# cbiffle/rtiow-rust

Hardware: AMD Instinct MI355X
Metric: Msamples/s (pixels*spp/s), book-1 random-spheres 1200x800 (higher is better)
Workload: dtype f32

## Files before the change

rtiow-rust_amd/capi.py:

```python
import ctypes as C
import math
import os
import time

import numpy as np

from . import noise

c_f32p = C.POINTER(C.c_float)
c_u32p = C.POINTER(C.c_uint32)
c_u8p = C.POINTER(C.c_uint8)

INVALID_ID = 0xFFFFFFFF
FLAG_COUNTERS = 1
FLAG_TRACE_KERNEL = 2
FLAG_PARTIAL = 4
FLAG_RESUME = 8
FLAG_SUM_SQUARES = 16
FLAG_SAMPLE_COUNTS = 32
FLAG_RETIRE = 64
RETIRE_MAX_RADIUS = 8
FLAG_DENOISE = 128
DENOISE_MAX_RADIUS = 8
DENOISE_MAX_PATCH = 3
# ... 471 lines not shown
        f("object_translate", C.c_uint32, [C.c_void_p, c_f32p, C.c_uint32])
        f("object_scale", C.c_uint32, [C.c_void_p, c_f32p, C.c_uint32])
        f("object_rotate_y", C.c_uint32, [C.c_void_p, C.c_float, C.c_uint32])
        f("object_and", C.c_uint32, [C.c_void_p, C.c_uint32, C.c_uint32])
        f("object_rect_prism", C.c_uint32, [C.c_void_p, c_f32p, c_f32p, C.c_uint32])
        f("object_linear_move", C.c_uint32, [C.c_void_p, C.c_uint32, c_f32p])
        f("object_constant_medium", C.c_uint32, [C.c_void_p, C.c_uint32, C.c_float, C.c_uint32])
        f("object_bvh", C.c_uint32, [C.c_void_p, c_u32p, C.c_size_t, C.c_float, C.c_float])
        f("object_bvh_sah", C.c_uint32, [C.c_void_p, c_u32p, C.c_size_t, C.c_float, C.c_float])
        f("camera_look", C.c_int, [c_f32p, c_f32p, c_f32p] + [C.c_float] * 6 + [C.POINTER(Camera)])
        f("scene_create", C.c_int, [C.c_void_p, c_u32p, C.c_size_t, C.c_int, C.POINTER(C.c_void_p)])
        f("scene_destroy", None, [C.c_void_p])
        self._declare_render()
        f("debug_hit_top", C.c_int, [C.c_void_p, C.c_size_t, c_f32p, C.c_uint64, C.c_float, c_f32p, c_u32p])
        f("debug_samples", C.c_int, [C.c_void_p, C.POINTER(Camera), C.POINTER(Params), C.c_size_t,
                                     c_u32p, c_u32p, c_u32p, c_f32p, c_u32p])
        f("debug_math", C.c_int, [C.c_int, C.c_int, C.c_size_t, c_f32p, c_f32p, c_f32p])
        f("tonemap", C.c_int, [C.c_int, C.c_size_t, c_f32p, c_u8p])

    def _declare_render(self):
        f = self._fn
        f("device_count", C.c_int, [C.POINTER(C.c_int)])
        f("scene_set_option", C.c_int, [C.c_void_p, C.c_char_p, C.c_int])
        f("scene_info", C.c_int, [C.c_void_p, c_u32p, c_u32p, c_u32p, C.POINTER(C.c_uint64), c_u32p])
        f("par_cast", C.c_int, [C.c_void_p, C.POINTER(Camera), C.POINTER(Params), c_f32p, C.POINTER(Stats)])
        f("par_cast_device", C.c_int, [C.c_void_p, C.POINTER(Camera), C.POINTER(Params), C.c_void_p,
                                       C.c_void_p, C.POINTER(Stats)])
        f("par_cast_multi", C.c_int, [C.POINTER(C.c_void_p), C.c_int, C.POINTER(Camera), C.POINTER(Params), c_f32p,
                                      C.POINTER(Stats)])
        f("multi_reset", C.c_int, [C.c_char_p, C.POINTER(C.c_uint64)])
        f("debug_flatten", C.c_int, [C.c_void_p, c_u32p, C.c_size_t, c_u32p, c_u32p, c_u32p, C.c_size_t])
        f("debug_flatten_pool2", C.c_int, [C.c_void_p, c_u32p, C.c_size_t, c_u32p, c_u32p, c_u32p, C.c_size_t])
        f("tonemap_device", C.c_int, [C.c_int, C.c_size_t, C.c_void_p, C.c_void_p, C.c_void_p])

    def _fn(self, name, restype, argtypes):
        try:
            fn = getattr(self.lib, self.prefix + name)
        except AttributeError:
            def fn(*_a, _n=self.prefix + name):
                raise RtError(ERR_INVALID, "%s: symbol %s is not exported by this build" % (self.path, _n))
            setattr(self, "_" + name, fn)
            return fn
        fn.restype = restype
        fn.argtypes = argtypes
        setattr(self, "_" + name, fn)
        return fn

    def last_error(self):
        return (self._last_error() or b"").decode()

    def check(self, code):
        if code != 0:
            raise RtError(code, self.last_error())

    def check_id(self, i):
        if i == INVALID_ID:
            raise RtError(-1, self.last_error())
        return i

    def builder(self):
        return Builder(self)

    def device_count(self):
        n = C.c_int(0)
        self.check(self._device_count(C.byref(n)))
        return n.value
# ... 129 lines not shown
    def rect_prism(self, p0, p1, material):
        return self.be.check_id(self.be._object_rect_prism(self.h, _f3(p0), _f3(p1), material))

    def linear_move(self, obj, motion):
        return self.be.check_id(self.be._object_linear_move(self.h, obj, _f3(motion)))

    def constant_medium(self, boundary, density, material):
        return self.be.check_id(self.be._object_constant_medium(self.h, boundary, density, material))

    def bvh(self, objs, exposure=(0.0, 1.0)):
        arr = (C.c_uint32 * max(1, len(objs)))(*objs)
        return self.be.check_id(self.be._object_bvh(self.h, arr, len(objs), exposure[0], exposure[1]))

    def flatten(self, world):
        arr = (C.c_uint32 * max(1, len(world)))(*world)
        n, feat = C.c_uint32(), C.c_uint32()
        self.be.check(self.be._debug_flatten(self.h, arr, len(world), C.byref(n), C.byref(feat), None, 0))
        words = np.zeros((n.value, 8), dtype=np.uint32)
        self.be.check(self.be._debug_flatten(self.h, arr, len(world), C.byref(n), C.byref(feat),
                                             words.ctypes.data_as(c_u32p), n.value))
        return words, feat.value

    def flatten_pool2(self, world):
        arr = (C.c_uint32 * max(1, len(world)))(*world)
        n = C.c_uint32()
        table = np.zeros(24, dtype=np.uint32)
        self.be.check(self.be._debug_flatten_pool2(self.h, arr, len(world), C.byref(n), table.ctypes.data_as(c_u32p), None, 0))
        words = np.zeros((n.value, 8), dtype=np.uint32)
        self.be.check(self.be._debug_flatten_pool2(self.h, arr, len(world), C.byref(n), table.ctypes.data_as(c_u32p),
                                                   words.ctypes.data_as(c_u32p), n.value))
        items = [tuple(int(v) for v in table[4 * k:4 * k + 4]) for k in range(int(table[20]))]
        return words, items, int(table[21]), int(table[22])

    def bvh_sah(self, objs, exposure=(0.0, 1.0)):
        arr = (C.c_uint32 * max(1, len(objs)))(*objs)
        return self.be.check_id(self.be._object_bvh_sah(self.h, arr, len(objs), exposure[0], exposure[1]))

    def scene(self, world, device=0):
        arr = (C.c_uint32 * max(1, len(world)))(*world)
        h = C.c_void_p()
        self.be.check(self.be._scene_create(self.h, arr, len(world), device, C.byref(h)))
        sc = self.be.scene_class(self.be, h, self)
        sc.apply_env_options()
        return sc


class Scene:
    def __init__(self, backend, handle, builder):
        self.be = backend
        self.h = handle
        self._builder = builder

    def close(self):
        if self.h:
            self.be._scene_destroy(self.h)
            self.h = None

    def __del__(self):
        try:
            self.close()
        except Exception:
            pass

    ENV_OPTIONS = ("kernel", "chunks", "lpt", "lpt_phase1", "lpt_deep", "lpt_shift", "ray_lds", "sync", "block", "wg_per_cu", "window",
                   "box_leave", "refill_min", "gather_min", "run_ahead", "run_ahead_min", "sphere_min", "verbose", "bvh4", "box_chains", "force_rccl", "multi_gather", "multi_planes", "scratch_mb", "frames_in_flight", "small_frames", "drain_share", "hoist", "deep_sized", "mat_lds", "pool2", "p2_refill", "p2_box_leave", "p2_park", "p2_sphere", "p2_prism", "p2_list", "p2_push")

    def set_option(self, name, value):
        self.be.check(self.be._scene_set_option(self.h, name.encode(), int(value)))

    def apply_env_options(self):
        if not hasattr(self.be, "_scene_set_option"):
            return
        for name in self.ENV_OPTIONS:
            v = os.environ.get("RTG_" + name.upper())
            if v is not None:
                self.set_option(name, int(v))

    def info(self):
        a, b, c, d, e = C.c_uint32(), C.c_uint32(), C.c_uint32(), C.c_uint64(), C.c_uint32()
        self.be.check(self.be._scene_info(self.h, C.byref(a), C.byref(b), C.byref(c), C.byref(d), C.byref(e)))
        return {"instructions": a.value, "materials": b.value, "textures": c.value, "hbm_bytes": d.value, "box_followers": e.value}

    def _par_cast_args(self, args, threads):
        return args

    def par_cast(self, camera, nx, ny, ns, seed=0xDEADBEEF, stats=False, out=None, threads=0, counts=None, counters=None,
                 retire=None, denoise=None, features=None, **kw):
        def call(p, buf):
            st = Stats.new()
            self.be.check(self.be._par_cast(*self._par_cast_args(
                [self.h, C.byref(camera), C.byref(p), buf.ctypes.data_as(c_f32p), C.byref(st)], threads)))
            return st
        return _render(lambda part: _supported(self.be, part), call, nx, ny, ns, seed, stats, out,
                       stats if counters is None else counters, counts, retire, denoise, features, kw, exact=True)

    def par_cast_device(self, camera, params, d_out_ptr, stream=None, want_stats=False, sample_begin=None, partial=None,
                        resume=None, squares=None, counts=None, retire=None, denoise=None, features=None):
        over = {"squares": squares, "counts": counts, "retire": retire, "denoise": denoise, "features": features}
# ... 245 lines not shown
```

rtiow-rust_amd/csrc/rtg_api.hip:

```cpp
#include <hip/hip_runtime.h>

#include <dlfcn.h>
#include <rccl/rccl.h>

#include <cmath>
#include <cstdio>
#include <cstdlib>
#include <cstring>
#include <map>
#include <mutex>
#include <functional>
#include <string>
#include <tuple>
#include <vector>

#include "../../include/rtiow_gpu.h"
#include "rt_pool.h"
#include "rt_retire.h"
#include "rt_denoise.h"
#include "rt_features.h"
#include "rt_multi_planes.h"
#include "rt_pool_full.h"
#include "rt_sync_full.h"
#include "rt_pool2.h"
#include "rt_trace.h"
#include "scene_builder.h"

using namespace rtg;

#include "rtg_kernels.inc"

namespace {
thread_local std::string g_err;

int fail(int code, const std::string& msg) {
  g_err = msg;
  return code;
}
int hip_fail(hipError_t e, const char* what) {
  return fail(RTG_ERR_DEVICE, std::string(what) + ": " + hipGetErrorString(e));
}
#define HIP_TRY(expr)                                   \
  do {                                                  \
    hipError_t e_ = (expr);                             \
    if (e_ != hipSuccess) return hip_fail(e_, #expr);   \
  } while (0)
}

struct rtg_builder {
  SceneBuilder sb;
// ... 9 lines not shown
  size_t stack_bytes = 0;
  uint32_t* d_slots = nullptr;
  size_t slots_bytes = 0;
  float* d_scratch = nullptr;
  size_t scratch_bytes = 0;
  LaunchConsts* d_consts = nullptr;
  uint32_t* d_lpt = nullptr;
  size_t lpt_bytes = 0;
  LptQueue lpt_desc{};
  KernelKind last_kernel = KernelKind::baseline;
  uint32_t last_pix_work = 0;
  uint32_t* d_list = nullptr;
  size_t list_bytes = 0;
  uint32_t* d_compact = nullptr;
  size_t compact_bytes = 0;
  unsigned long long counts_samples = 0;
  void* d_retire = nullptr;
  size_t retire_bytes = 0;
  const char* refusal = nullptr;
  void* d_denoise = nullptr;
  size_t denoise_bytes = 0;
  rtg_denoise denoise_in{};
  uint32_t* d_features = nullptr;
  size_t features_bytes = 0;
  rtg_features features_in{};
};

struct rtg_scene {
  int device = 0;
  DevScene dev{};
  uint32_t features = 0;
  uint32_t n_prog = 0, n_mat = 0, n_tex = 0;
  uint64_t bytes = 0;
  void* buffers[13] = {nullptr, nullptr, nullptr, nullptr, nullptr, nullptr, nullptr, nullptr, nullptr, nullptr, nullptr, nullptr, nullptr};
  const uint32_t* d_parent = nullptr;
  hipStream_t own_stream = nullptr;
  int num_cus = 0;
  float* d_frame = nullptr;
  size_t frame_bytes = 0;
  int force_chunks = 0;
  uint64_t scratch_limit = 0;
  bool whole_scratch = false;
  int verbose = 0;
  int window = -1;
  int ray_lds = 1;
  int force_rccl = 0;
  int multi_gather = 0;
  float* d_pack = nullptr;
  size_t pack_bytes = 0;
  float* d_recv = nullptr;
  size_t recv_bytes = 0;
  int multi_planes = 0;
  hipEvent_t post0 = nullptr, post1 = nullptr;
  hipEvent_t pack0 = nullptr, pack1 = nullptr, unpack0 = nullptr;
  int bvh4 = 0;
  uint32_t wide_bytes = 0;
  int box_chains = 1;
  uint32_t n_followers = 0;
  const uint32_t* d_chain_off = nullptr;
  uint32_t chain_bytes = 0;
  int sync_full = -1;
  uint32_t n_box = 0;
  int lpt = 2;
  int lpt_deep = 4;
  int lpt_shift = 0;
  int lpt_phase1 = 0;
  int kernel_version = 3;
  PoolTuning pool_tune{40, 16, 24, 16, 16, 40};
  PoolTuning full_tune{20, 24, 32, 16, 24, 40};
  PoolTuning sync_tune{20, 16, 32, 16, 16, 40};
  int wg_per_cu = 0;
  int full_threads = 0;
  int pool_threads = 0;
  int mat_lds = 1;
  int deep_sized = 1;
  int hoist = 1;
  uint32_t seg_first = 0, seg_end = 0;
  int drain_share = 1;
  int pool2 = 1;
  uint32_t n_prog2 = 0, n_box2 = 0;
  DevScene dev2{};
  const P2Table* d_p2 = nullptr;
  Pool2Tuning pool2_tune{24, 48, 40, 4, 8, 24, 2};
  int guide_lds = 0;
  int small_frames = 1;
  LaunchCtx ctx[RTG_MAX_FRAMES];
  int n_ctx = 1, next_ctx = 0;
  LaunchCtx* cx = &ctx[0];
};

static void ctx_free_buffers(LaunchCtx* c) {
  if (c->busy) (void)hipEventSynchronize(c->done);
  c->busy = false;
// ... 311 lines not shown
  float theta = fov * 3.14159265358979323846f / 180.f;
  float half_height = tanf(theta / 2.f);
  float half_width = aspect * half_height;
  float w[3] = {from[0] - at[0], from[1] - at[1], from[2] - at[2]};
  unit(w);
  float u[3], v[3];
  cross3(up, w, u);
  unit(u);
  cross3(w, u, v);
  float hw_fd = half_width * focus_dist, hh_fd = half_height * focus_dist;
  float h2 = (2.f * half_width) * focus_dist, v2 = (2.f * half_height) * focus_dist;
  for (int i = 0; i < 3; i++) {
    out->origin[i] = from[i];
    out->lower_left_corner[i] = ((from[i] - hw_fd * u[i]) - hh_fd * v[i]) - focus_dist * w[i];
    out->horizontal[i] = h2 * u[i];
    out->vertical[i] = v2 * v[i];
    out->u[i] = u[i];
    out->v[i] = v[i];
  }
  out->lens_radius = lens_radius;
  out->exposure_start = e0;
  out->exposure_end = e1;
  return RTG_OK;
}

static int upload(void** dst, const void* src, size_t bytes, uint64_t* total) {
  size_t alloc = bytes ? bytes : 16;
  HIP_TRY(hipMalloc(dst, alloc));
  if (bytes) HIP_TRY(hipMemcpy(*dst, src, bytes, hipMemcpyHostToDevice));
  *total += alloc;
  return RTG_OK;
}

void rtg_scene_destroy(rtg_scene* s) {
  if (!s) return;
  (void)hipSetDevice(s->device);
  for (void* p : s->buffers)
    if (p) (void)hipFree(p);
  for (LaunchCtx& c : s->ctx) {
    ctx_free_buffers(&c);
    if (c.d_counters) (void)hipFree(c.d_counters);
    if (c.d_consts) (void)hipFree(c.d_consts);
    if (c.ev0) (void)hipEventDestroy(c.ev0);
    if (c.ev1) (void)hipEventDestroy(c.ev1);
    if (c.done) (void)hipEventDestroy(c.done);
  }
  if (s->d_frame) (void)hipFree(s->d_frame);
  if (s->d_pack) (void)hipFree(s->d_pack);
  if (s->d_recv) (void)hipFree(s->d_recv);
  if (s->post0) (void)hipEventDestroy(s->post0);
  if (s->post1) (void)hipEventDestroy(s->post1);
  for (hipEvent_t ev : {s->pack0, s->pack1, s->unpack0})
    if (ev) (void)hipEventDestroy(ev);
  if (s->own_stream) (void)hipStreamDestroy(s->own_stream);
  delete s;
}

int rtg_scene_create(rtg_builder* b, const rtg_id* world, size_t n, int device, rtg_scene** out) {
  if (!b || !out || (!world && n)) return fail(RTG_ERR_INVALID, "null argument");
  FlatScene fs;
  try {
    b->sb.flatten(world, n, &fs);
  } catch (const BuildError& e) {
    return fail(e.code, e.msg);
  }
  int ndev = 0;
// ... 45 lines not shown
  if (!fs.hi2.empty()) {
    if ((rc = upload(&s->buffers[9], fs.lo2.data(), fs.lo2.size() * 16, &s->bytes)) ||
        (rc = upload(&s->buffers[10], fs.hi2.data(), fs.hi2.size() * 16, &s->bytes)) ||
        (rc = upload(&s->buffers[11], &fs.p2, sizeof(P2Table), &s->bytes))) {
      rtg_scene_destroy(s);
      return rc;
    }
    s->dev2 = s->dev;
    s->dev2.lo = (const uint4*)s->buffers[9], s->dev2.hi = (const uint4*)s->buffers[10];
    s->dev2.n_prog = s->n_prog2 = (uint32_t)fs.hi2.size();
    s->dev2.lds_off = nullptr, s->dev2.lds_image_bytes = 0;
    s->d_p2 = (const P2Table*)s->buffers[11];
    for (const Packet& h : fs.hi2) s->n_box2 += (h.w[3] & 0xffu) == OP_BOX ? 1u : 0u;
  }
  if ((fs.features & (FEAT_ALL | FEAT_BOUNDARY)) == 0) {
    std::vector<uint32_t> ops(fs.hi.size()), off(fs.hi.size());
    for (size_t i = 0; i < fs.hi.size(); i++) ops[i] = fs.hi[i].w[3];
    s->dev.lds_image_bytes = lds_image_offsets(ops.data(), ops.size(), off.data());
    if ((rc = upload(&s->buffers[6], off.data(), off.size() * sizeof(uint32_t), &s->bytes))) {
      rtg_scene_destroy(s);
      return rc;
    }
    s->dev.lds_off = (const uint32_t*)s->buffers[6];
    std::vector<uint8_t> follower(fs.hi.size());
    s->n_followers = box_chain_followers(reinterpret_cast<const uint32_t (*)[4]>(fs.lo.data()), reinterpret_cast<const uint32_t (*)[4]>(fs.hi.data()), fs.hi.size(), follower.data());
    if (s->n_followers) {
      s->chain_bytes = lds_image_offsets(ops.data(), ops.size(), off.data(), follower.data());
      if ((rc = upload(&s->buffers[12], off.data(), off.size() * sizeof(uint32_t), &s->bytes))) {
        rtg_scene_destroy(s);
        return rc;
      }
      s->d_chain_off = (const uint32_t*)s->buffers[12];
    }
    std::vector<uint32_t> wide;
    if (build_wide_image(fs.lo.data(), fs.hi.data(), fs.hi.size(), wide)) {
      if ((rc = upload(&s->buffers[7], wide.data(), wide.size() * sizeof(uint32_t), &s->bytes))) {
        rtg_scene_destroy(s);
        return rc;
      }
      s->wide_bytes = (uint32_t)(wide.size() * sizeof(uint32_t));
    }
  }
  hipDeviceProp_t prop;
  if (hipGetDeviceProperties(&prop, device) == hipSuccess) s->num_cus = prop.multiProcessorCount;
  if (s->num_cus <= 0) s->num_cus = 256;
  if ((rc = ctx_acquire(s))) {
    rtg_scene_destroy(s);
    return rc;
  }
  s->next_ctx = 0;
  *out = s;
  return RTG_OK;
}


int rtg_scene_set_option(rtg_scene* s, const char* name, int value) {
  if (!s || !name) return fail(RTG_ERR_INVALID, "null argument");
  const std::string k(name);
  const uint32_t u = (uint32_t)value;
  if (k == "kernel") s->kernel_version = value;
  else if (k == "chunks") s->force_chunks = value;
  else if (k == "scratch_mb") s->scratch_limit = value > 0 ? (uint64_t)value << 20 : 0;
  else if (k == "lpt") s->lpt = value;
  else if (k == "lpt_phase1") s->lpt_phase1 = value;
  else if (k == "lpt_deep") s->lpt_deep = value;
  else if (k == "lpt_shift") s->lpt_shift = std::min(6, std::max(0, value));
  else if (k == "ray_lds") s->ray_lds = value;
  else if (k == "box_chains") s->box_chains = value;
  else if (k == "bvh4") {
    if (value && !s->wide_bytes) return fail(RTG_ERR_INVALID, "bvh4: the scene is not one Bvh of spheres (no 4-wide image)");
    if (value && pool_lds_bytes(s->wide_bytes, s->n_mat, (uint32_t)(s->pool_threads > 0 ? s->pool_threads : RT_POOL_MAX_THREADS) / 64u, true, false) > 160 * 1024)
      return fail(RTG_ERR_INVALID, "bvh4: the 4-wide image does not fit a CU's 160 KB of LDS (the 4-wide walk only exists LDS-staged)");
    s->bvh4 = value;
  }
  else if (k == "frames_in_flight") {
    if (value < 1 || value > RTG_MAX_FRAMES) return fail(RTG_ERR_INVALID, "frames_in_flight: 1 .. 4");
    HIP_TRY(hipSetDevice(s->device));
    for (int i = value; i < RTG_MAX_FRAMES; i++) ctx_free_buffers(&s->ctx[i]);
    s->n_ctx = value, s->next_ctx = 0;
  }
  else if (k == "force_rccl") s->force_rccl = value;
  else if (k == "multi_gather") s->multi_gather = value;
  else if (k == "multi_planes") s->multi_planes = value;
  else if (k == "sync") s->sync_full = value;
  else if (k == "block") {
    if (value < 64 || value > 1024 || value % 64) return fail(RTG_ERR_INVALID, "block: a multiple of 64 in [64, 1024]");
    s->pool_threads = s->full_threads = value;
  }
  else if (k == "wg_per_cu") s->wg_per_cu = value;
  else if (k == "drain_share") s->drain_share = value;
  else if (k == "hoist") s->hoist = value;
  else if (k == "pool2") s->pool2 = value;
  else if (k == "deep_sized") s->deep_sized = value;
  else if (k == "mat_lds") s->mat_lds = value;
  else if (k == "guide_lds") s->guide_lds = value;
  else if (k == "small_frames") s->small_frames = value;
  else if (k == "verbose") s->verbose = value;
  else if (k == "window") s->window = value;
  else if (k == "box_leave") s->pool_tune.box_leave = s->full_tune.box_leave = s->sync_tune.box_leave = u;
  else if (k == "refill_min") s->pool_tune.refill_min = s->full_tune.refill_min = s->sync_tune.refill_min = u;
  else if (k == "gather_min") s->pool_tune.gather_min = s->full_tune.gather_min = s->sync_tune.gather_min = u;
// ... 296 lines not shown
```

rtiow-rust_amd/csrc/rtg_launch.inc:

```
static uint64_t scratch_cap(int n_ctx) {
  size_t free_b = 0, total_b = 0;
  if (hipMemGetInfo(&free_b, &total_b) != hipSuccess) return (16ull << 30) / (uint64_t)std::max(1, n_ctx);
  return (uint64_t)free_b / 2 / (uint64_t)std::max(1, n_ctx);
}

static uint32_t samples_per_pass(const rtg_scene* s, uint64_t pix_work, uint32_t ns) {
  const uint64_t per_sample = pix_work * 3 * sizeof(float);
  uint64_t budget = s->scratch_limit ? s->scratch_limit : std::max<uint64_t>(scratch_cap(s->n_ctx), s->cx->scratch_bytes);
  if (s->whole_scratch) budget = ~0ull;
  uint64_t k = std::max<uint64_t>(1, budget / std::max<uint64_t>(per_sample, 1));
  k = std::min<uint64_t>(k, 0xfffffffeull / std::max<uint64_t>(pix_work, 1));
  k = std::max<uint64_t>(1, std::min<uint64_t>(k, ns));
  const uint64_t n_pass = (ns + k - 1) / k;
  return (uint32_t)((ns + n_pass - 1) / n_pass);
}

static uint64_t rank_pix_work(const DevParams& d) {
  const uint32_t tiles_x = (d.nx + d.tile_w - 1) / d.tile_w, tiles_y = (d.ny + d.tile_h - 1) / d.tile_h, tiles = tiles_x * tiles_y;
  const uint32_t owned = tiles > d.rank ? (tiles - d.rank + d.nranks - 1) / d.nranks : 0;
  return ((uint64_t)owned * d.tile_w * d.tile_h + 255u) & ~255ull;
}
static uint64_t owned_pixels(const DevParams& d) {
  uint64_t px = 0;
  uint32_t tiles_x = (d.nx + d.tile_w - 1) / d.tile_w, tiles_y = (d.ny + d.tile_h - 1) / d.tile_h;
// ... 110 lines not shown
    }
  }
  return hipSuccess;
}

template <bool COUNT>
static hipError_t launch_pool(rtg_scene* s, const DevCamera& cam, const DevParams& d, float* d_out,
                              hipStream_t stream, const SampleSlice& sl) {
  const uint64_t pix_work = sl.counts ? sl.list_work : rank_pix_work(d);
  if (pix_work == 0) return hipSuccess;
  if (pix_work > 0xfffffffeull) return hipErrorInvalidValue;
  const uint32_t ns_call = d.ns - sl.begin;
  uint64_t n_chunks = ns_call;
  if (s->force_chunks > 0) n_chunks = (uint64_t)s->force_chunks;
  if (n_chunks > ns_call) n_chunks = ns_call;
  const bool use_scratch = n_chunks > 1 || sl.sliced() || sl.squares || sl.counts;
  uint32_t per_pass = d.ns, chunk = d.ns;
  if (use_scratch) {
    per_pass = samples_per_pass(s, pix_work, ns_call);
    chunk = (uint32_t)((ns_call + n_chunks - 1) / n_chunks);
    if (per_pass < ns_call || sl.begin % chunk != 0u || sl.squares || sl.counts) chunk = 1u;
    hipError_t ea = grow((void**)&s->cx->d_scratch, &s->cx->scratch_bytes, pix_work * per_pass * 3 * sizeof(float));
    if (ea != hipSuccess) return ea;
  }
  s->cx->last_pix_work = use_scratch && per_pass == d.ns ? (uint32_t)pix_work : 0u;
  uint32_t* queue = (uint32_t*)(s->cx->d_counters + 7);
  const uint64_t work0 = pix_work * (use_scratch ? (std::min(ns_call, per_pass) + chunk - 1) / chunk : 1u);
  const PoolGeometry geo = pool_geometry(s, work0, RT_POOL_MAX_THREADS, s->pool_threads, POOL, true);
  const int bt = geo.bt;
  const uint32_t waves = (uint32_t)bt / 64;
  const size_t lds_limit = 160 * 1024;
  const bool wide = s->bvh4 && s->wide_bytes != 0 && !sl.counts;
  const bool chains = !COUNT && !wide && s->box_chains && s->d_chain_off != nullptr;
  DevScene dev = s->dev;
  if (wide) dev.lds_off = (const uint32_t*)s->buffers[7], dev.lds_image_bytes = s->wide_bytes;
  if (chains) dev.lds_off = s->d_chain_off, dev.lds_image_bytes = s->chain_bytes;
  const uint32_t image = dev.lds_image_bytes;
  bool use_lds = image != 0 && pool_lds_bytes(image, s->n_mat, waves, true, false) <= lds_limit;
  if (wide && !use_lds) return hipErrorNotSupported;
  bool ray_lds = s->ray_lds && pool_lds_bytes(image, s->n_mat, waves, use_lds, true) <= lds_limit && (!use_lds || image < (1u << 17));
  size_t lds = pool_lds_bytes(image, s->n_mat, waves, use_lds, ray_lds);
  if (s->verbose && s->ray_lds && !ray_lds && use_lds && image >= (1u << 17) && pool_lds_bytes(image, s->n_mat, waves, use_lds, true) <= lds_limit)
    fprintf(stderr, "[rtg] pool: the LDS image is %u B (>= 128 KB): the slots' hot fields stay in global memory although they would fit LDS (their 16-bit best_pc holds image offsets / 8 < 2^14)\n", image);
  void (*kernel)(DevScene, const LaunchConsts*, float*, uint32_t, uint32_t*, unsigned long long*, PoolTuning, uint32_t*);
  if (sl.counts) {
    if (ray_lds) kernel = use_lds ? render_lean_pool<true, COUNT, true, false, true> : render_lean_pool<false, COUNT, true, false, true>;
    else kernel = use_lds ? render_lean_pool<true, COUNT, false, false, true> : render_lean_pool<false, COUNT, false, false, true>;
  } else if (wide) kernel = ray_lds ? render_lean_pool<true, COUNT, true, true> : render_lean_pool<true, COUNT, false, true>;
  else if (ray_lds) kernel = use_lds ? render_lean_pool<true, COUNT, true> : render_lean_pool<false, COUNT, true>;
  else kernel = use_lds ? render_lean_pool<true, COUNT, false> : render_lean_pool<false, COUNT, false>;
  if (s->verbose && chains && use_lds)
    fprintf(stderr, "[rtg] pool: box chains: %u follower record(s) dropped from the LDS image (%u B, full image %u B)\n",
            s->n_followers, s->chain_bytes, s->dev.lds_image_bytes);
  PoolLaunch L{KernelKind::lean_pool, bt, 0, lds, geo, POOL};
  hipError_t e = kernel_setup(s, (const void*)kernel, bt, lds, &L.per_cu);
  if (e != hipSuccess) return e;
  auto chunks = [&](uint32_t s0, uint32_t end) {
    ChunkMode cm{};
    cm.scratch = nullptr, cm.chunk = d.ns, cm.n_chunks = 1, cm.pix_work = (uint32_t)pix_work, cm.s_begin = s0;
    if (use_scratch) {
      cm.chunk = chunk;
      cm.n_chunks = (end - s0 + chunk - 1) / chunk;
      cm.scratch = s->cx->d_scratch - 3ull * s0 * pix_work;
    }
    return cm;
  };
  auto issue = [&](uint32_t s0, const DevParams& dp, const ChunkMode& cm, uint32_t grid, uint32_t total_work) {
    if (s->verbose)
      fprintf(stderr, "[rtg] pool: samples [%u, %u) of %u: grid %u x %d threads, %d WG/CU, lds %zu B (program staged: %d, hot slot fields in LDS: %d), %u chunk(s) of %u samples, cost-ordered queue after %u chunk(s)\n",
              s0, dp.ns, d.ns, grid, bt, L.per_cu, lds, (int)use_lds, (int)ray_lds, cm.n_chunks, cm.chunk, (cm.lpt_samples - (cm.lpt_samples ? s0 : 0u)) / (cm.chunk ? cm.chunk : 1u));
    hipError_t eg = grow((void**)&s->cx->d_slots, &s->cx->slots_bytes, (size_t)grid * waves * POOL * POOL_FIELDS * sizeof(uint32_t));
    if (eg != hipSuccess) return eg;
    launch_pass_setup(s, LaunchConsts{cam, dp, cm, make_pixmap(dp)}, queue, stream);
    hipLaunchKernelGGL(kernel, dim3(grid), dim3(bt), lds, stream, dev, (const LaunchConsts*)s->cx->d_consts, d_out, total_work, queue,
                       s->cx->d_counters, s->pool_tune, s->cx->d_slots);
    return hipSuccess;
  };
  return sample_passes(s, d, d_out, stream, sl, L, per_pass, chunks, issue);
}

static bool build_wide_image(const Packet* lo, const Packet* hi, size_t n, std::vector<uint32_t>& out) {
  struct T { uint32_t box; int left, right; uint32_t sphere; };
  std::vector<T> nodes;
  auto op_of = [&](size_t i) { return hi[i].w[3] & 0xffu; };
  if (n < 4 || op_of(n - 1) != OP_END || op_of(0) != OP_BOX || hi[0].w[2] != n - 1) return false;
  bool ok = true;
// ... 490 lines not shown
```

rtiow-rust_amd/csrc/rtg_probes.inc:

```
int rtg_debug_hit_top(rtg_scene* s, size_t n, const float* rays, uint64_t seed, float t_near, float* out,
                      uint32_t* out_material) {
  if (!s || !rays || !out || !out_material) return fail(RTG_ERR_INVALID, "null argument");
  HIP_TRY(hipSetDevice(s->device));
  DevBuf<float> d_rays, d_out;
  DevBuf<uint32_t> d_mat;
  HIP_TRY(d_rays.alloc(7 * n));
  HIP_TRY(d_out.alloc(8 * n));
  HIP_TRY(d_mat.alloc(n));
  HIP_TRY(hipMemcpy(d_rays.p, rays, 7 * n * sizeof(float), hipMemcpyHostToDevice));
  dim3 grid((uint32_t)((n + 63) / 64)), block(64);
  if (n) {
    if (s->features & FEAT_DEEP)
      hipLaunchKernelGGL((debug_hit_top_kernel<FEAT_ALL | FEAT_DEEP>), grid, block, 0, 0, s->dev, (uint32_t)n, d_rays.p, (uint32_t)seed,
                         (uint32_t)(seed >> 32), t_near, d_out.p, d_mat.p);
    else if (s->features == 0)
      hipLaunchKernelGGL((debug_hit_top_kernel<0u>), grid, block, 0, 0, s->dev, (uint32_t)n, d_rays.p, (uint32_t)seed,
                         (uint32_t)(seed >> 32), t_near, d_out.p, d_mat.p);
    else
      hipLaunchKernelGGL((debug_hit_top_kernel<FEAT_ALL>), grid, block, 0, 0, s->dev, (uint32_t)n, d_rays.p,
                         (uint32_t)seed, (uint32_t)(seed >> 32), t_near, d_out.p, d_mat.p);
  }
  HIP_TRY(hipGetLastError());
  HIP_TRY(hipDeviceSynchronize());
  HIP_TRY(hipMemcpy(out, d_out.p, 8 * n * sizeof(float), hipMemcpyDeviceToHost));
// ... 121 lines not shown
  if (features) *features = fs.features;
  if (words_out) {
    size_t m = fs.lo.size() < capacity ? fs.lo.size() : capacity;
    for (size_t i = 0; i < m; i++) {
      std::memcpy(words_out + 8 * i, fs.lo[i].w, 16);
      std::memcpy(words_out + 8 * i + 4, fs.hi[i].w, 16);
    }
  }
  return RTG_OK;
}

int rtg_debug_flatten_pool2(rtg_builder* b, const rtg_id* world, size_t n, uint32_t* n_instructions, uint32_t* table_out,
                            uint32_t* words_out, size_t capacity) {
  if (!b || (!world && n)) return fail(RTG_ERR_INVALID, "null argument");
  FlatScene fs;
  try {
    b->sb.flatten(world, n, &fs);
  } catch (const BuildError& e) {
    return fail(e.code, e.msg);
  }
  if (n_instructions) *n_instructions = (uint32_t)fs.lo2.size();
  static_assert(sizeof(P2Table) == 24 * sizeof(uint32_t), "rtg_debug_flatten_pool2: table_out holds 24 words");
  if (table_out) std::memcpy(table_out, &fs.p2, sizeof(P2Table));
  if (words_out) {
    size_t m = fs.lo2.size() < capacity ? fs.lo2.size() : capacity;
    for (size_t i = 0; i < m; i++) {
      std::memcpy(words_out + 8 * i, fs.lo2[i].w, 16);
      std::memcpy(words_out + 8 * i + 4, fs.hi2[i].w, 16);
    }
  }
  return RTG_OK;
}

int rtg_debug_math(int device, int op, size_t n, const float* in, const float* in2, float* out) {
  if (!in || !out || op < 0 || op > 5 || (op == 5 && !in2)) return fail(RTG_ERR_INVALID, "bad argument");
  int ndev = 0;
  if (hipGetDeviceCount(&ndev) != hipSuccess || device < 0 || device >= ndev) return fail(RTG_ERR_DEVICE, "no HIP device");
  HIP_TRY(hipSetDevice(device));
  DevBuf<float> di, di2, dout;
  HIP_TRY(di.alloc(n));
  HIP_TRY(di2.alloc(n));
  HIP_TRY(dout.alloc(n));
  HIP_TRY(hipMemcpy(di.p, in, n * sizeof(float), hipMemcpyHostToDevice));
  if (in2) HIP_TRY(hipMemcpy(di2.p, in2, n * sizeof(float), hipMemcpyHostToDevice));
  if (n) hipLaunchKernelGGL(debug_math_kernel, dim3((uint32_t)((n + 255) / 256)), dim3(256), 0, 0, op, n, di.p, di2.p, dout.p);
  HIP_TRY(hipGetLastError());
  HIP_TRY(hipDeviceSynchronize());
  HIP_TRY(hipMemcpy(out, dout.p, n * sizeof(float), hipMemcpyDeviceToHost));
  return RTG_OK;
}
```

rtiow-rust_amd/roofline.py:

```python
import json
import os

N_CUS = 256
SIMDS_PER_CU = 4
NOMINAL_CLOCK_HZ = 2.4e9
ISSUE_CYCLES = 2.0
HBM_PEAK_GBS = 8000.0
XCDS = 8


def source_stamp(root):
    import hashlib
    csrc = os.path.join(root, "rtiow-rust_amd", "csrc")
    files = sorted(f for f in os.listdir(csrc) if f.endswith((".h", ".inc", ".hip", ".cpp")) or f == "Makefile")
    files = [os.path.join("rtiow-rust_amd", "csrc", f) for f in files] + [os.path.join("include", "rtiow_gpu.h")]
    blobs = {}
    for rel in files:
        data = open(os.path.join(root, rel), "rb").read()
        blobs[rel] = hashlib.sha1(b"blob %d\0" % len(data) + data).hexdigest()
    digest = hashlib.sha1("".join("%s %s\n" % (k, v) for k, v in sorted(blobs.items())).encode()).hexdigest()
    return {"digest": digest, "blobs": blobs}


def profile_staleness(pmc, root, lib_override=None, knobs=None):
    st = pmc.get("build")
    if not st:
        return "the profile carries no build stamp (collected before round 3)"
    if lib_override:
        return "RTIOW_GPU_LIB points at another build of the library (%s)" % lib_override
    now = source_stamp(root)
    if st.get("digest") != now["digest"]:
        changed = sorted(k for k in set(now["blobs"]) | set(st.get("blobs", {})) if now["blobs"].get(k) != st.get("blobs", {}).get(k))
        return "kernel sources changed since the counters were collected: " + ", ".join(os.path.basename(c) for c in changed)
    if knobs:
        return "schedule options differ from the profiled run: " + ", ".join(knobs)
    return None


def load_pmc(path):
    with open(path) as f:
        return json.load(f)


def shader_clock_hz(pmc, kernel_s_profiled=None):
    c = pmc.get("counters_avg_per_launch", {})
    if kernel_s_profiled and c.get("GRBM_GUI_ACTIVE"):
        return c["GRBM_GUI_ACTIVE"] / XCDS / kernel_s_profiled
    return None
# ... 100 lines not shown
```

Measured before the change: 7034.

## Prune always-passed interior BVH boxes from the LDS program image

Adds a host-side box plan that fires a few hundred random bounce rays through the flattened BVH program. It marks interior box records that every probe passed and whose children are leaf or prunable boxes, then builds an LDS offset table that drops them. The renderer uses this table by default (box_prune=1), so rays skip box tests that almost always succeed and the LDS image gets smaller. The risk is that the probes are a statistical sample: a pruned box that some real rays would have missed now costs extra child tests. The plan also adds build-time work and an extra device buffer.

```diff
diff --git a/include/rtiow_gpu_debug.h b/include/rtiow_gpu_debug.h
--- /dev/null
+++ b/include/rtiow_gpu_debug.h
@@ -0,0 +1,14 @@
+#ifndef RTIOW_GPU_DEBUG_H
+#define RTIOW_GPU_DEBUG_H
+#include "rtiow_gpu.h"
+#ifdef __cplusplus
+extern "C" {
+#endif
+
+int rtg_debug_box_plan(rtg_builder* b, const rtg_id* world, size_t n, const uint32_t* words, size_t n_records,
+                       uint8_t* mask_out, size_t capacity);
+
+#ifdef __cplusplus
+}
+#endif
+#endif
diff --git a/rtiow-rust_amd/capi.py b/rtiow-rust_amd/capi.py
--- a/rtiow-rust_amd/capi.py
+++ b/rtiow-rust_amd/capi.py
@@ -527,6 +527,7 @@
         f("debug_flatten", C.c_int, [C.c_void_p, c_u32p, C.c_size_t, c_u32p, c_u32p, c_u32p, C.c_size_t])
         f("debug_flatten_pool2", C.c_int, [C.c_void_p, c_u32p, C.c_size_t, c_u32p, c_u32p, c_u32p, C.c_size_t])
         f("tonemap_device", C.c_int, [C.c_int, C.c_size_t, C.c_void_p, C.c_void_p, C.c_void_p])
+        f("debug_box_plan", C.c_int, [C.c_void_p, c_u32p, C.c_size_t, c_u32p, C.c_size_t, c_u8p, C.c_size_t])
 
     def _fn(self, name, restype, argtypes):
         try:
@@ -722,6 +723,22 @@
         items = [tuple(int(v) for v in table[4 * k:4 * k + 4]) for k in range(int(table[20]))]
         return words, items, int(table[21]), int(table[22])
 
+    def box_plan(self, world=None, words=None):
+        if words is not None:
+            words = np.ascontiguousarray(words, dtype=np.uint32)
+            mask = np.zeros(len(words), dtype=np.uint8)
+            n = self.be._debug_box_plan(None, None, 0, words.ctypes.data_as(c_u32p), len(words), mask.ctypes.data_as(c_u8p), len(mask))
+        else:
+            arr = (C.c_uint32 * max(1, len(world)))(*world)
+            n = self.be._debug_box_plan(self.h, arr, len(world), None, 0, None, 0)
+            if n < 0:
+                self.be.check(n)
+            mask = np.zeros(n, dtype=np.uint8)
+            n = self.be._debug_box_plan(self.h, arr, len(world), None, 0, mask.ctypes.data_as(c_u8p), len(mask))
+        if n < 0:
+            self.be.check(n)
+        return mask
+
     def bvh_sah(self, objs, exposure=(0.0, 1.0)):
         arr = (C.c_uint32 * max(1, len(objs)))(*objs)
         return self.be.check_id(self.be._object_bvh_sah(self.h, arr, len(objs), exposure[0], exposure[1]))
@@ -753,7 +770,7 @@
             pass
 
     ENV_OPTIONS = ("kernel", "chunks", "lpt", "lpt_phase1", "lpt_deep", "lpt_shift", "ray_lds", "sync", "block", "wg_per_cu", "window",
-                   "box_leave", "refill_min", "gather_min", "run_ahead", "run_ahead_min", "sphere_min", "verbose", "bvh4", "box_chains", "force_rccl", "multi_gather", "multi_planes", "scratch_mb", "frames_in_flight", "small_frames", "drain_share", "hoist", "deep_sized", "mat_lds", "pool2", "p2_refill", "p2_box_leave", "p2_park", "p2_sphere", "p2_prism", "p2_list", "p2_push")
+                   "box_leave", "refill_min", "gather_min", "run_ahead", "run_ahead_min", "sphere_min", "verbose", "bvh4", "box_chains", "box_prune", "force_rccl", "multi_gather", "multi_planes", "scratch_mb", "frames_in_flight", "small_frames", "drain_share", "hoist", "deep_sized", "mat_lds", "pool2", "p2_refill", "p2_box_leave", "p2_park", "p2_sphere", "p2_prism", "p2_list", "p2_push")
 
     def set_option(self, name, value):
         self.be.check(self.be._scene_set_option(self.h, name.encode(), int(value)))
diff --git a/rtiow-rust_amd/csrc/rt_box_plan.h b/rtiow-rust_amd/csrc/rt_box_plan.h
--- /dev/null
+++ b/rtiow-rust_amd/csrc/rt_box_plan.h
@@ -0,0 +1,250 @@
+#pragma once
+#include <cmath>
+#include <cstddef>
+#include <cstdint>
+#include <cstring>
+#include <vector>
+
+#include "flat_scene.h"
+
+namespace rtg {
+
+constexpr uint8_t BOX_KEPT = 0, BOX_FOLLOWER = 1, BOX_PRUNED = 2;
+#ifndef RT_BOX_PLAN_PROBES
+#define RT_BOX_PLAN_PROBES 256
+#endif
+#ifndef RT_BOX_PLAN_FULL
+#define RT_BOX_PLAN_FULL 0
+#endif
+constexpr uint32_t BOX_PLAN_PROBES = RT_BOX_PLAN_PROBES;
+constexpr bool BOX_PLAN_FULL = RT_BOX_PLAN_FULL != 0;
+
+struct BoxPlan {
+  uint32_t n_pruned = 0;
+  uint32_t n_sure = 0;
+  uint32_t n_rays = 0;
+};
+
+namespace box_plan_detail {
+inline float as_f(uint32_t u) {
+  float f;
+  std::memcpy(&f, &u, 4);
+  return f;
+}
+inline bool aabb_hit(const uint32_t* lo, const uint32_t* hi, const float* o, const float* inv, float t_near, float best) {
+  const float mn[3] = {as_f(lo[0]), as_f(lo[2]), as_f(hi[0])}, mx[3] = {as_f(lo[1]), as_f(lo[3]), as_f(hi[1])};
+  float t0[3], t1[3];
+  for (int a = 0; a < 3; a++) {
+    const float u = (mn[a] - o[a]) * inv[a], v = (mx[a] - o[a]) * inv[a];
+    t0[a] = inv[a] < 0.f ? v : u, t1[a] = inv[a] < 0.f ? u : v;
+  }
+  const float start = fmaxf(t_near, fmaxf(fmaxf(t0[0], t0[1]), t0[2]));
+  const float end = fminf(best, fminf(fminf(t1[0], t1[1]), t1[2]));
+  return end > start;
+}
+inline bool sphere_hit(const uint32_t* lo, uint32_t flags, const float* o, const float* d, float dd, float t_near, float best, float* t_out) {
+  float p[3] = {o[0], o[1], o[2]};
+  if (flags & F_TRANSLATE)
+    for (int a = 0; a < 3; a++) p[a] = o[a] - as_f(lo[a]);
+  const float r = as_f(lo[3]);
+  const float b = p[0] * d[0] + p[1] * d[1] + p[2] * d[2];
+  const float c = p[0] * p[0] + p[1] * p[1] + p[2] * p[2] - r * r;
+  const float disc = b * b - dd * c;
+  if (disc > 0.f) {
+    const float sq = sqrtf(disc);
+    float t = (-b - sq) / dd;
+    if (t < best && t >= t_near) return *t_out = t, true;
+    t = (-b + sq) / dd;
+    if (t < best && t >= t_near) return *t_out = t, true;
+  }
+  return false;
+}
+struct Rng {
+  uint64_t s;
+  uint64_t next() {
+    uint64_t z = (s += 0x9e3779b97f4a7c15ull);
+    z = (z ^ (z >> 30)) * 0xbf58476d1ce4e5b9ull;
+    z = (z ^ (z >> 27)) * 0x94d049bb133111ebull;
+    return z ^ (z >> 31);
+  }
+  float unit() { return (float)(next() >> 40) * (1.f / 16777216.f); }
+  void in_unit_sphere(float* v) {
+    do {
+      for (int a = 0; a < 3; a++) v[a] = 2.f * unit() - 1.f;
+    } while (v[0] * v[0] + v[1] * v[1] + v[2] * v[2] >= 1.f);
+  }
+};
+}
+
+inline BoxPlan box_plan(const uint32_t (*lo)[4], const uint32_t (*hi)[4], size_t n, const uint8_t* follower, uint8_t* mask,
+                        uint8_t* sure = nullptr, uint32_t n_probes = BOX_PLAN_PROBES) {
+  using namespace box_plan_detail;
+  BoxPlan out;
+  for (size_t j = 0; j < n; j++) {
+    mask[j] = follower && follower[j] ? BOX_FOLLOWER : BOX_KEPT;
+    if (sure) sure[j] = 0;
+  }
+  auto op = [&](size_t j) { return hi[j][3] & 0xffu; };
+  auto skip = [&](size_t j) { return (size_t)hi[j][2]; };
+  if (n < 4 || n > 0x7fffffffu) return out;
+  std::vector<int32_t> parent(n, -1);
+  std::vector<uint32_t> depth(n, 0);
+  {
+    std::vector<uint32_t> open;
+    for (size_t j = 0; j < n; j++) {
+      while (!open.empty() && skip(open.back()) <= j) open.pop_back();
+      if (!open.empty()) parent[j] = (int32_t)open.back(), depth[j] = (uint32_t)open.size();
+      if (op(j) != OP_BOX) continue;
+      if (skip(j) <= j || skip(j) >= n || (!open.empty() && skip(j) > skip(open.back()))) return out;
+      open.push_back((uint32_t)j);
+    }
+  }
+  auto leaf_box = [&](size_t j) { return op(j) == OP_BOX && j + 2 < n && op(j + 1) == OP_SPHERE && skip(j) == j + 2; };
+  auto finite6 = [&](size_t j) {
+    return std::isfinite(as_f(lo[j][0])) && std::isfinite(as_f(lo[j][1])) && std::isfinite(as_f(lo[j][2])) &&
+           std::isfinite(as_f(lo[j][3])) && std::isfinite(as_f(hi[j][0])) && std::isfinite(as_f(hi[j][1]));
+  };
+  auto contains = [&](size_t j, size_t c) {
+    return as_f(lo[j][0]) <= as_f(lo[c][0]) && as_f(lo[j][1]) >= as_f(lo[c][1]) && as_f(lo[j][2]) <= as_f(lo[c][2]) &&
+           as_f(lo[j][3]) >= as_f(lo[c][3]) && as_f(hi[j][0]) <= as_f(hi[c][0]) && as_f(hi[j][1]) >= as_f(hi[c][1]);
+  };
+  std::vector<uint8_t> prunable(n, 0);
+  uint32_t n_prunable = 0;
+  for (size_t j = n; j-- > 0;) {
+    if (op(j) != OP_BOX || j + 1 >= n || op(j + 1) != OP_BOX) continue;
+    const size_t L = j + 1, R = skip(L);
+    if (!(L < R && R < skip(j)) || op(R) != OP_BOX || skip(R) != skip(j)) continue;
+    if (!finite6(j) || !finite6(L) || !finite6(R) || !contains(j, L) || !contains(j, R)) continue;
+    if (!(leaf_box(L) || prunable[L]) || !(leaf_box(R) || prunable[R])) continue;
+    prunable[j] = 1, n_prunable++;
+  }
+  if (!n_prunable) return out;
+  std::vector<uint8_t> choosable(prunable);
+  for (size_t j = 0; j + 1 < n; j++) {
+    if (!prunable[j] || !follower) continue;
+    size_t k = j + 1;
+    while (k + 1 < n && follower[k] && !leaf_box(k)) k++;
+    if (follower[k] && leaf_box(k)) choosable[j] = 0;
+  }
+
+  std::vector<uint64_t> n_pass(n, 0);
+  std::vector<uint32_t> spheres, starts;
+  for (size_t j = 0; j < n; j++)
+    if (op(j) == OP_SPHERE) spheres.push_back((uint32_t)j);
+  auto centre = [&](uint32_t j, float* c) {
+    for (int a = 0; a < 3; a++) c[a] = (hi[j][3] & F_TRANSLATE) ? as_f(lo[j][a]) : 0.f;
+  };
+  float cmin[3] = {INFINITY, INFINITY, INFINITY}, cmax[3] = {-INFINITY, -INFINITY, -INFINITY};
+  for (uint32_t j : spheres) {
+    float c[3];
+    centre(j, c);
+    for (int a = 0; a < 3; a++) cmin[a] = fminf(cmin[a], c[a]), cmax[a] = fmaxf(cmax[a], c[a]);
+  }
+  std::vector<uint8_t> enclosing(n, 0);
+  for (uint32_t j : spheres) {
+    float cj[3];
+    centre(j, cj);
+    const float r = as_f(lo[j][3]);
+    float far2 = 0.f;
+    for (int a = 0; a < 3; a++) {
+      const float d = fmaxf(cmax[a] - cj[a], cj[a] - cmin[a]);
+      far2 += d * d;
+    }
+    const bool all = spheres.size() > 1 && far2 < r * r;
+    enclosing[j] = all;
+    if (!all && std::isfinite(r) && std::isfinite(cj[0]) && std::isfinite(cj[1]) && std::isfinite(cj[2])) starts.push_back(j);
+  }
+  uint64_t n_rays = 0;
+  if (!starts.empty()) {
+    Rng rng{0x626f78706c616e31ull ^ (uint64_t)n};
+    const float t_near = 0.001f;
+    while (n_rays < n_probes) {
+      const uint32_t s0 = starts[rng.next() % starts.size()];
+      float c[3], nrm[3], o[3], d[3], v[3];
+      centre(s0, c);
+      do rng.in_unit_sphere(nrm);
+      while (nrm[0] * nrm[0] + nrm[1] * nrm[1] + nrm[2] * nrm[2] < 1e-4f);
+      const float len = sqrtf(nrm[0] * nrm[0] + nrm[1] * nrm[1] + nrm[2] * nrm[2]), r0 = as_f(lo[s0][3]);
+      for (int a = 0; a < 3; a++) nrm[a] /= len, o[a] = c[a] + r0 * nrm[a];
+      const uint32_t bounces = 1u + (uint32_t)(rng.next() % 3u);
+      for (uint32_t k = 0; k <= bounces && n_rays < n_probes; k++) {
+        rng.in_unit_sphere(v);
+        for (int a = 0; a < 3; a++) d[a] = nrm[a] + v[a];
+        const float inv[3] = {1.f / d[0], 1.f / d[1], 1.f / d[2]};
+        const float dd = d[0] * d[0] + d[1] * d[1] + d[2] * d[2];
+        float best = 3.402823466e+38f;
+        int64_t best_pc = -1;
+        n_rays++;
+        for (size_t pc = 0; pc < n;) {
+          const uint32_t o_ = op(pc);
+          if (o_ == OP_BOX) {
+            if (aabb_hit(lo[pc], hi[pc], o, inv, t_near, best)) n_pass[pc]++, pc++;
+            else pc = skip(pc);
+          } else if (o_ == OP_SPHERE) {
+            float t;
+            if (sphere_hit(lo[pc], hi[pc][3], o, d, dd, t_near, best, &t)) best = t, best_pc = (int64_t)pc;
+            pc++;
+          } else break;
+        }
+        if (best_pc < 0 || enclosing[best_pc]) break;
+        centre((uint32_t)best_pc, c);
+        const float r = as_f(lo[best_pc][3]);
+        for (int a = 0; a < 3; a++) o[a] = o[a] + best * d[a], nrm[a] = (o[a] - c[a]) / r;
+        if (!(std::isfinite(nrm[0]) && std::isfinite(nrm[1]) && std::isfinite(nrm[2]))) break;
+      }
+    }
+  }
+  out.n_rays = (uint32_t)n_rays;
+
+  uint64_t states = 0;
+  for (size_t j = 0; BOX_PLAN_FULL && j < n; j++)
+    if (op(j) == OP_BOX) states += depth[j] + 2u;
+  const bool dp = BOX_PLAN_FULL && states <= (1ull << 26);
+  std::vector<uint32_t> kidx(n, 0);
+  std::vector<uint8_t> pruned(n, 0);
+  if (dp) {
+    std::vector<std::vector<uint64_t>> acc(n);
+    std::vector<std::vector<uint8_t>> choice(n);
+    std::vector<uint64_t> path_pass;
+    for (size_t j = n; j-- > 0;) {
+      if (op(j) != OP_BOX) continue;
+      const uint32_t dj = depth[j];
+      if (acc[j].empty()) acc[j].assign(dj + 2u, 0);
+      path_pass.assign(dj + 1u, n_rays);
+      for (int32_t a = parent[j], k = (int32_t)dj; a >= 0; a = parent[a], k--) path_pass[k] = n_pass[a];
+      std::vector<uint64_t> f(dj + 1u);
+      choice[j].assign(dj + 1u, 0);
+      for (uint32_t k = 0; k <= dj; k++) {
+        const uint64_t own = follower && follower[j] ? 0u : path_pass[k];
+        const uint64_t keep = own + acc[j][dj + 1u], leave = acc[j][k];
+        if (choosable[j] && leave <= keep) f[k] = leave, choice[j][k] = 1;
+        else f[k] = keep;
+      }
+      std::vector<uint64_t>().swap(acc[j]);
+      if (parent[j] >= 0) {
+        std::vector<uint64_t>& up = acc[parent[j]];
+        if (up.empty()) up.assign(dj + 1u, 0);
+        for (uint32_t k = 0; k <= dj; k++) up[k] += f[k];
+      }
+    }
+    for (size_t j = 0; j < n; j++) {
+      if (op(j) != OP_BOX) continue;
+      const int32_t p = parent[j];
+      kidx[j] = p < 0 ? 0u : (pruned[p] ? kidx[p] : depth[j]);
+      pruned[j] = choice[j][kidx[j]];
+    }
+  } else {
+    for (size_t j = 0; j < n; j++) pruned[j] = choosable[j] && n_rays && n_pass[j] == n_rays;
+  }
+  for (size_t j = 0; j < n; j++) {
+    if (!pruned[j] || mask[j] == BOX_FOLLOWER) continue;
+    mask[j] = BOX_PRUNED, out.n_pruned++;
+    if (n_pass[j] == n_rays) {
+      out.n_sure++;
+      if (sure) sure[j] = 1;
+    }
+  }
+  return out;
+}
+
+}
diff --git a/rtiow-rust_amd/csrc/rtg_api.hip b/rtiow-rust_amd/csrc/rtg_api.hip
--- a/rtiow-rust_amd/csrc/rtg_api.hip
+++ b/rtiow-rust_amd/csrc/rtg_api.hip
@@ -3,6 +3,7 @@
 #include <dlfcn.h>
 #include <rccl/rccl.h>
 
+#include <chrono>
 #include <cmath>
 #include <cstdio>
 #include <cstdlib>
@@ -15,7 +16,9 @@
 #include <vector>
 
 #include "../../include/rtiow_gpu.h"
+#include "../../include/rtiow_gpu_debug.h"
 #include "rt_pool.h"
+#include "rt_box_plan.h"
 #include "rt_retire.h"
 #include "rt_denoise.h"
 #include "rt_features.h"
@@ -91,7 +94,7 @@
   uint32_t features = 0;
   uint32_t n_prog = 0, n_mat = 0, n_tex = 0;
   uint64_t bytes = 0;
-  void* buffers[13] = {nullptr, nullptr, nullptr, nullptr, nullptr, nullptr, nullptr, nullptr, nullptr, nullptr, nullptr, nullptr, nullptr};
+  void* buffers[15] = {};
   const uint32_t* d_parent = nullptr;
   hipStream_t own_stream = nullptr;
   int num_cus = 0;
@@ -118,6 +121,13 @@
   uint32_t n_followers = 0;
   const uint32_t* d_chain_off = nullptr;
   uint32_t chain_bytes = 0;
+  int box_prune = 1;
+  uint32_t n_pruned = 0;
+  float plan_ms = 0.f;
+  const uint32_t* d_prune_off[2] = {nullptr, nullptr};
+  uint32_t prune_bytes[2] = {0, 0};
+  std::vector<uint32_t> plan_ops;
+  std::vector<uint8_t> plan_mask;
   int sync_full = -1;
   uint32_t n_box = 0;
   int lpt = 2;
@@ -495,6 +505,19 @@
   return RTG_OK;
 }
 
+static int prune_table(rtg_scene* s, int chains) {
+  if (s->d_prune_off[chains] || !s->n_pruned) return RTG_OK;
+  const size_t n = s->plan_mask.size();
+  std::vector<uint8_t> drop(n);
+  std::vector<uint32_t> off(n);
+  for (size_t i = 0; i < n; i++) drop[i] = s->plan_mask[i] == BOX_PRUNED || (chains && s->plan_mask[i] == BOX_FOLLOWER);
+  s->prune_bytes[chains] = lds_image_offsets(s->plan_ops.data(), n, off.data(), drop.data());
+  int rc = upload(&s->buffers[13 + chains], off.data(), n * sizeof(uint32_t), &s->bytes);
+  if (rc) return rc;
+  s->d_prune_off[chains] = (const uint32_t*)s->buffers[13 + chains];
+  return RTG_OK;
+}
+
 void rtg_scene_destroy(rtg_scene* s) {
   if (!s) return;
   (void)hipSetDevice(s->device);
@@ -606,6 +629,19 @@
       }
       s->d_chain_off = (const uint32_t*)s->buffers[12];
     }
+    if (s->dev.lds_image_bytes - LDS_BOX_BYTES * (s->n_box / 2u) <= 160u * 1024u) {
+      s->plan_mask.resize(fs.hi.size());
+      const auto t0 = std::chrono::steady_clock::now();
+      s->n_pruned = box_plan(reinterpret_cast<const uint32_t (*)[4]>(fs.lo.data()), reinterpret_cast<const uint32_t (*)[4]>(fs.hi.data()), fs.hi.size(), follower.data(), s->plan_mask.data()).n_pruned;
+      s->plan_ms = std::chrono::duration<float, std::milli>(std::chrono::steady_clock::now() - t0).count();
+      if (s->n_pruned) {
+        s->plan_ops = ops;
+        if ((rc = prune_table(s, 1))) {
+          rtg_scene_destroy(s);
+          return rc;
+        }
+      }
+    }
     std::vector<uint32_t> wide;
     if (build_wide_image(fs.lo.data(), fs.hi.data(), fs.hi.size(), wide)) {
       if ((rc = upload(&s->buffers[7], wide.data(), wide.size() * sizeof(uint32_t), &s->bytes))) {
@@ -640,7 +676,18 @@
   else if (k == "lpt_deep") s->lpt_deep = value;
   else if (k == "lpt_shift") s->lpt_shift = std::min(6, std::max(0, value));
   else if (k == "ray_lds") s->ray_lds = value;
-  else if (k == "box_chains") s->box_chains = value;
+  else if (k == "box_chains") {
+    if (!value) {
+      HIP_TRY(hipSetDevice(s->device));
+      int rc = prune_table(s, 0);
+      if (rc) return rc;
+    }
+    s->box_chains = value;
+  }
+  else if (k == "box_prune") {
+    if (value < 0 || value > 2) return fail(RTG_ERR_INVALID, "box_prune: 0 .. 2");
+    s->box_prune = value;
+  }
   else if (k == "bvh4") {
     if (value && !s->wide_bytes) return fail(RTG_ERR_INVALID, "bvh4: the scene is not one Bvh of spheres (no 4-wide image)");
     if (value && pool_lds_bytes(s->wide_bytes, s->n_mat, (uint32_t)(s->pool_threads > 0 ? s->pool_threads : RT_POOL_MAX_THREADS) / 64u, true, false) > 160 * 1024)
diff --git a/rtiow-rust_amd/csrc/rtg_launch.inc b/rtiow-rust_amd/csrc/rtg_launch.inc
--- a/rtiow-rust_amd/csrc/rtg_launch.inc
+++ b/rtiow-rust_amd/csrc/rtg_launch.inc
@@ -166,9 +166,11 @@
   const size_t lds_limit = 160 * 1024;
   const bool wide = s->bvh4 && s->wide_bytes != 0 && !sl.counts;
   const bool chains = !COUNT && !wide && s->box_chains && s->d_chain_off != nullptr;
+  const bool prune = !wide && s->box_prune && (!COUNT || s->box_prune == 2) && s->d_prune_off[s->box_chains ? 1 : 0] != nullptr;
   DevScene dev = s->dev;
   if (wide) dev.lds_off = (const uint32_t*)s->buffers[7], dev.lds_image_bytes = s->wide_bytes;
   if (chains) dev.lds_off = s->d_chain_off, dev.lds_image_bytes = s->chain_bytes;
+  if (prune) dev.lds_off = s->d_prune_off[s->box_chains ? 1 : 0], dev.lds_image_bytes = s->prune_bytes[s->box_chains ? 1 : 0];
   const uint32_t image = dev.lds_image_bytes;
   bool use_lds = image != 0 && pool_lds_bytes(image, s->n_mat, waves, true, false) <= lds_limit;
   if (wide && !use_lds) return hipErrorNotSupported;
@@ -183,9 +185,10 @@
   } else if (wide) kernel = ray_lds ? render_lean_pool<true, COUNT, true, true> : render_lean_pool<true, COUNT, false, true>;
   else if (ray_lds) kernel = use_lds ? render_lean_pool<true, COUNT, true> : render_lean_pool<false, COUNT, true>;
   else kernel = use_lds ? render_lean_pool<true, COUNT, false> : render_lean_pool<false, COUNT, false>;
-  if (s->verbose && chains && use_lds)
-    fprintf(stderr, "[rtg] pool: box chains: %u follower record(s) dropped from the LDS image (%u B, full image %u B)\n",
-            s->n_followers, s->chain_bytes, s->dev.lds_image_bytes);
+  if (s->verbose && (chains || prune) && use_lds)
+    fprintf(stderr, "[rtg] pool: box chains: %u follower record(s)%s, box pruning: %u interior record(s)%s (plan %.2f ms): LDS image %u B, %u records of %u; without followers %u B, full image %u B\n",
+            s->n_followers, s->box_chains ? " dropped" : " kept", s->n_pruned, prune ? " dropped" : " kept", s->plan_ms, image,
+            s->n_prog - (s->box_chains ? s->n_followers : 0u) - (prune ? s->n_pruned : 0u), s->n_prog, s->chain_bytes ? s->chain_bytes : s->dev.lds_image_bytes, s->dev.lds_image_bytes);
   PoolLaunch L{KernelKind::lean_pool, bt, 0, lds, geo, POOL};
   hipError_t e = kernel_setup(s, (const void*)kernel, bt, lds, &L.per_cu);
   if (e != hipSuccess) return e;
diff --git a/rtiow-rust_amd/csrc/rtg_probes.inc b/rtiow-rust_amd/csrc/rtg_probes.inc
--- a/rtiow-rust_amd/csrc/rtg_probes.inc
+++ b/rtiow-rust_amd/csrc/rtg_probes.inc
@@ -177,6 +177,39 @@
   return RTG_OK;
 }
 
+int rtg_debug_box_plan(rtg_builder* b, const rtg_id* world, size_t n, const uint32_t* words, size_t n_records, uint8_t* mask_out,
+                       size_t capacity) {
+  std::vector<Packet> lo, hi;
+  bool lean = true;
+  if (words) {
+    lo.resize(n_records), hi.resize(n_records);
+    for (size_t i = 0; i < n_records; i++) {
+      std::memcpy(lo[i].w, words + 8 * i, 16), std::memcpy(hi[i].w, words + 8 * i + 4, 16);
+      const uint32_t op = hi[i].w[3] & 0xffu;
+      lean = lean && (op == OP_BOX || op == OP_SPHERE || op == OP_END) && !(hi[i].w[3] & F_MOVE);
+      if (op == OP_BOX && hi[i].w[2] >= n_records) return fail(RTG_ERR_INVALID, "rtg_debug_box_plan: a skip pointer leaves the program");
+    }
+  } else {
+    if (!b || (!world && n)) return fail(RTG_ERR_INVALID, "null argument");
+    FlatScene fs;
+    try {
+      b->sb.flatten(world, n, &fs);
+    } catch (const BuildError& e) {
+      return fail(e.code, e.msg);
+    }
+    lean = (fs.features & (FEAT_ALL | FEAT_BOUNDARY)) == 0;
+    lo.swap(fs.lo), hi.swap(fs.hi);
+  }
+  if (hi.size() > 0x7fffffffu) return fail(RTG_ERR_INVALID, "rtg_debug_box_plan: program too large");
+  std::vector<uint8_t> follower(hi.size(), 0), mask(hi.size(), 0);
+  if (lean && !hi.empty()) {
+    box_chain_followers(reinterpret_cast<const uint32_t (*)[4]>(lo.data()), reinterpret_cast<const uint32_t (*)[4]>(hi.data()), hi.size(), follower.data());
+    box_plan(reinterpret_cast<const uint32_t (*)[4]>(lo.data()), reinterpret_cast<const uint32_t (*)[4]>(hi.data()), hi.size(), follower.data(), mask.data());
+  }
+  if (mask_out) std::memcpy(mask_out, mask.data(), std::min(mask.size(), capacity));
+  return (int)hi.size();
+}
+
 int rtg_debug_math(int device, int op, size_t n, const float* in, const float* in2, float* out) {
   if (!in || !out || op < 0 || op > 5 || (op == 5 && !in2)) return fail(RTG_ERR_INVALID, "bad argument");
   int ndev = 0;
diff --git a/rtiow-rust_amd/roofline.py b/rtiow-rust_amd/roofline.py
--- a/rtiow-rust_amd/roofline.py
+++ b/rtiow-rust_amd/roofline.py
@@ -13,7 +13,7 @@
     import hashlib
     csrc = os.path.join(root, "rtiow-rust_amd", "csrc")
     files = sorted(f for f in os.listdir(csrc) if f.endswith((".h", ".inc", ".hip", ".cpp")) or f == "Makefile")
-    files = [os.path.join("rtiow-rust_amd", "csrc", f) for f in files] + [os.path.join("include", "rtiow_gpu.h")]
+    files = [os.path.join("rtiow-rust_amd", "csrc", f) for f in files] + [os.path.join("include", f) for f in sorted(os.listdir(os.path.join(root, "include"))) if f.endswith(".h")]
     blobs = {}
     for rel in files:
         data = open(os.path.join(root, rel), "rb").read()
```

New measurement: 7281, median of 6. 1.04x the previous value.
